# xmlyqing00/V-FloodNet

Hardware: AMD Instinct MI355X
Metric: segmented frames/sec at 480p (higher is better)
Workload: dtype f32

## Files before the change

### include/vfn_hip.h

```cpp
#ifndef VFN_HIP_H
#define VFN_HIP_H

#ifdef __cplusplus
extern "C" {
#endif

#define VFN_ABI_VERSION 18
enum { VFN_DESC_CONV = 0, VFN_DESC_STEM = 1, VFN_DESC_BANKSCAN = 2, VFN_DESC_MEMREAD = 3, VFN_DESC_BANK = 4, VFN_DESC_WGRAD = 5,
       VFN_DESC_REFRESH_FILTER = 6, VFN_DESC_REFRESH_EPILOGUE = 7, VFN_DESC_GATHER = 8, VFN_DESC_BANKMATCH = 9,
       VFN_DESC_TRAIN_AUG = 10 };
int vfn_abi_version(void);
int vfn_sizeof_desc(int which);

typedef struct vfn_conv_desc {
    const float* in;
    const float* w;
    const float* scale;
    const float* shift;
    const float* res;
    float* out;
    int N, H, W, Cin, in_ld;
    int Ho, Wo, Cout, cout_pad, out_ld, res_ld;
    int KH, KW, stride, pad;
    int relu_in, relu_out;
// ... 125 lines not shown
    const float* var;
    float* scale;
    float* shift;
    float eps;
    int C;
} vfn_refresh_epilogue;
int vfn_refresh_elems_per_block(void);
int vfn_refresh_filters_f32(const vfn_refresh_filter* table_dev, int n, int total_blocks, void* stream);
int vfn_refresh_epilogues_f32(const vfn_refresh_epilogue* table_dev, int n, void* stream);
typedef struct vfn_gather_entry {
    const float* src;
    long long dst_offset;
    long long stride[4];
    int shape[4];
    int block0;
    int reserved;
} vfn_gather_entry;
int vfn_gather_strided_f32(const vfn_gather_entry* table_dev, int n, int total_blocks, float* dst, void* stream);
int vfn_dilate2_f32(const float* g, float* out, int N, int Ho, int Wo, int H, int W, int C, void* stream);
int vfn_bn_param_grads_f32(const float* g, const float* y, const float* idn, const float* beta, const float* gamma, int M, int C,
                           float* partial, int nb, float* dgamma, float* dbeta, void* stream);
int vfn_bn_param_grads_acc_f32(const float* g, const float* y, const float* idn, const float* beta, const float* gamma, int M, int C,
                               float* partial, int nb, float* dgamma, float* dbeta, int accumulate, int* counter,
                               void* stream);
int vfn_maxpool3x3s2_backward_f32(const float* x, const float* g, float* gx, int N, int H, int W, int C, const float* add, int relu_mask,
                                  void* stream);
int vfn_softmax_cols_f32(const float* S, int B, int Q, int ld, float scale, float* P, void* stream);
int vfn_softmax_cols_backward_f32(const float* P, const float* dP, int B, int Q, int ld, float scale, float* dS, void* stream);
int vfn_adamw_f32(float* p, const float* g, float* m, float* v, long long n, double lr, double beta1, double beta2, double eps,
                  double weight_decay, int step, void* stream);
int vfn_colsum_f32(const float* x, int M, int C, int ld, float* partial, int nb, float* out, void* stream);
#define VFN_COLSUM_COUNTERS 64
int vfn_colsum_acc_f32(const float* x, int M, int C, int ld, float* partial, int nb, float* out, int accumulate, int* counter,
                       void* stream);
int vfn_upsample2x_add_backward_f32(const float* gm, float* gs, float* gpm, int N, int h, int w, int C, int s_bcast,
                                    void* stream);
int vfn_segment_loss_f32(const float* logit, const int* label, int bs, int obj_n, int n, float lu, float* partial, float* stats,
                         float* grad, void* stream);
int vfn_segment_uncertainty_backward_f32(const float* logit, int bs, int obj_n, int n, const float* g_unc_dev,
                                         const float* g_scores, float* partial, float* stats, float* grad, void* stream);
int vfn_tail_grad_o_f32(const float* G, const float* p_up, const float* unc, const float* conf, const float* q, float* g_o,
                        int obj_n, int h, int w, int pad_top, int pad_left, int H0, int W0, void* stream);
int vfn_tail_split_f32(const float* g_p2, const float* unc, const float* conf, const float* q, float* g_q, float* g_cf, float* g_u,
                       int obj_n, int npix, void* stream);
int vfn_local_stats_backward_f32(const float* g_lm, const float* lm, const float* g_cf, const float* g_u, const float* g_p2,
                                 const float* r1, const float* rough, const float* p_up, float* dA, float* dBv, int* amax,
                                 float* g_r1, float* g_pup, int obj_n, int h, int w, int C, void* stream);

typedef struct vfn_bankscan_desc {
    const float* q;
    const float* bank_k;
    const int* bank_len;
    const float* rowscale;
    float* part;
    long long stride_q, stride_k, stride_rs;
    float scale;
    int ldq, q_per_obj, HW, obj_n, nsplit, mode;
    int precision;
    int* work_counter;
    const void* bank_k_lp;
    float* scores;
    long long stride_scores;
} vfn_bankscan_desc;

typedef struct vfn_memread_desc {
    const float* q;
    const float* qv;
    const float* bank_k;
    const float* bank_v;
    const int* bank_len;
    const float* ml;
    float* o_part;
    int* cnt;
    float* info;
    float* out;
    long long stride_k, stride_v, stride_cnt, stride_info;
    float scale, thres;
    int ldq, ldqv, ld_out, HW, obj_n, nsplit;
    int precision;
    const void* bank_k_lp;
    const void* bank_v_lp;
    const float* scores;
    long long stride_scores;
} vfn_memread_desc;

int vfn_bank_scan(const vfn_bankscan_desc* d, void* stream);
int vfn_bank_scan_finish(const float* part, int nsplit, int HW, int obj_n, int mode, float* ml, int* idx,
                         float* corr, const float* colscale, void* stream);
int vfn_memread_apply(const vfn_memread_desc* d, void* stream);

typedef struct vfn_bankmatch_desc {
    const float* q;
    const float* bank_k;
    const void* bank_k_lp;
    const int* bank_len;
    const float* rowscale;
    const float* qnorm;
    const float* colscale;
    float* part_x3;
    float* part_f32;
    int* ulist;
    int* ucount;
    int* utotal;
    int* work_counter;
    int* match_idx;
    float* match_corr;
    long long stride_q, stride_k, stride_rs;
    int ldq, HW, obj_n;
    int nsplit;
    int nsplit_fb;
} vfn_bankmatch_desc;
int vfn_bank_match_certified(const vfn_bankmatch_desc* d, void* stream);
int vfn_memread_finish(const vfn_memread_desc* d, void* stream);

#define VFN_BANK_MAX_HW 32768
typedef struct vfn_bank_desc {
    float* bank_k;
    float* bank_v;
    float* info;
    float* scratch_k;
    float* scratch_v;
    float* scratch_info;
    const int* bank_len;
    int* bank_len_rw;
    const float* bank_knorm;
    const float* bank_vnorm;
    const int* match_idx;
    const float* match_corr;
    const float* new_k;
    const float* new_knorm;
    const float* new_vnorm;
    int* app_pos;
    int* keep_dst;
    int* plan;
    int* stats;
    long long stride_k, stride_v, stride_info, stride_n, stride_new;
    double class_budget;
    float thres_close, update_rate, new_hit_init;
    int frame_idx, ld_new, voff, HW, obj_n, cap;
    int rm_class;
    int rm_request;
} vfn_bank_desc;

int vfn_bank_refresh_lp(const vfn_bank_desc* d, void* bank_k_lp, void* bank_v_lp, int all_rows, void* stream);
int vfn_bank_refresh_lp_keys(const vfn_bank_desc* d, void* bank_k_lp, int all_rows, void* stream);

int vfn_row_norms(const float* x, long long stride_obj, int ld, int dim, const int* len_dev, int rows,
                  int obj_n, float* nrm, float* inv , long long stride_n, void* stream);
int vfn_bank_merge(const vfn_bank_desc* d, void* stream);
int vfn_bank_append(const vfn_bank_desc* d, void* stream);
int vfn_bank_remove(const vfn_bank_desc* d, void* stream);
int vfn_bank_refresh_norms(const vfn_bank_desc* d, float* bank_knorm, float* bank_kinv, float* bank_vnorm, void* stream);
int vfn_scatter_mean_f32(const float* src, long long src_s0, long long src_s1, const long long* index,
                         int S, float* out, long long out_s0, long long out_s1, int D, void* stream);
int vfn_scatter_mean_checked_f32(const float* src, long long src_s0, long long src_s1, const long long* index,
                                 long long index_s0, int S, float* out, long long out_s0, long long out_s1, int D,
                                 long long B, int* status, void* stream);

int vfn_resize_bicubic_f32(const float* in, float* out, int C, int Hi, int Wi, int Ho, int Wo, void* stream);
int vfn_resize_nearest_f32(const float* in, float* out, int C, int Hi, int Wi, int Ho, int Wo, void* stream);
int vfn_softmax_objects_f32(const float* score, float* prob, int obj_n, int n, void* stream);
int vfn_resize_argmax_u8(const float* prob, unsigned char* label, int obj_n, int Hi, int Wi, int Ho, int Wo,
                         void* stream);
int vfn_postprocess_pred_u8(const unsigned char* pred_host, int H, int W, unsigned char* out_host);
int vfn_postprocess_pred_device_u8(const unsigned char* pred, unsigned char* out, int* scratch, int H, int W,
                                   void* stream);
// ... 111 lines not shown
```

### v-floodnet_amd/csrc/memory_read.hip

```cpp
#include "common.h"
#include "../../include/vfn_hip.h"
#include <type_traits>
#include <cstdlib>

namespace {

constexpr int DK = 128, DV = 512;
constexpr int CH = 64;

__device__ __forceinline__ int swz(int row, int chunk) { return row * DK + ((chunk ^ (row & 15)) << 2); }

__device__ __forceinline__ int swz64(int row, int chunk) { return row * CH + ((chunk ^ (row & 15)) << 2); }

__device__ __forceinline__ void chunk_load_async(float* sK, const float* src, int valid, int wave, int lane) {
#pragma unroll
    for (int j = 0; j < 8; ++j) {
        const int r = (wave * 8 + j) * 2 + (lane >> 5);
        const int pc = lane & 31;
        const int rr = min(r, valid - 1);
        const float* g = src + (size_t)rr * DK + ((pc ^ (r & 15)) << 2);
        __builtin_amdgcn_global_load_lds(g, sK + (wave * 8 + j) * 2 * DK, 16, 0, 0);
    }
}

// ... 1331 lines not shown
    }

    PH_DECL;
    for (int c = c_lo; c < c_hi; ++c) {
        const int b0 = c * CH;
        const bool more = c + 1 < c_hi;

        f32x16 acc;
        score_tile(sK, sQ, wr, wq, li, lh, acc);
        PH_MARK(0);

        const int rloc = wr * 32 + 4 * lh;
        const int mycnt = softmax_hits(acc, p.scale, qm, qinv, p.thres, B - b0, rloc);
#pragma unroll
        for (int g = 0; g < 4; ++g) {
            const int brow = rloc + 8 * g;
            const f32x4 v = {acc[4 * g], acc[4 * g + 1], acc[4 * g + 2], acc[4 * g + 3]};
            *reinterpret_cast<f32x4*>(sP + swz64(qcol, brow >> 2)) = v;
        }
        if (p.cnt && lh == 0 && mycnt > 0) {
            const int row = b0 + wr * 32 + li;
            if (row < B) atomicAdd(p.cnt + (size_t)obj * p.stride_cnt + row, mycnt);
        }
        PH_MARK(1);
        __syncthreads();
        PH_MARK(2);
        if (more) chunk_load_async8(sK, K + (size_t)(b0 + CH) * DK, min(CH, B - b0 - CH), wave, lane);

        f32x2 vb[3][4];
        const __amdgpu_buffer_rsrc_t vrsrc = __builtin_amdgcn_make_buffer_rsrc(
            const_cast<float*>(V + (size_t)b0 * DV), 0, min(CH, B - b0) * DV * 4, 0x00020000);
        auto load_v = [&](int kk, int slot) {
#pragma unroll
            for (int t = 0; t < 4; ++t)
                vb[slot][t] = __builtin_bit_cast(f32x2, __builtin_amdgcn_raw_buffer_load_b64(vrsrc, vlane_off + (unsigned)((8 * kk + t) * DV * 4), 0, 0));
        };
        load_v(0, 0);
        load_v(1, 1);
        __builtin_amdgcn_sched_barrier(0);
#pragma unroll
        for (int kk = 0; kk < CH / 8; ++kk) {
            const int cur = kk % 3;
            if (kk + 2 < CH / 8) load_v(kk + 2, (kk + 2) % 3);
            __builtin_amdgcn_sched_barrier(0);
            const int lc = 2 * kk + lh;
            f32x4 a[4];
#pragma unroll
            for (int tq = 0; tq < 4; ++tq) a[tq] = *reinterpret_cast<const f32x4*>(sP + swz64(tq * 32 + li, lc));
#pragma unroll
            for (int t = 0; t < 4; ++t)
#pragma unroll
                for (int tq = 0; tq < 4; ++tq) {
                    o[tq][0] = __builtin_amdgcn_mfma_f32_32x32x2f32(a[tq][t], vb[cur][t][0], o[tq][0], 0, 0, 0);
                    o[tq][1] = __builtin_amdgcn_mfma_f32_32x32x2f32(a[tq][t], vb[cur][t][1], o[tq][1], 0, 0, 0);
                }
        }
        PH_MARK(3);
        __syncthreads();
        PH_MARK(4);
    }
#ifdef VFN_CENSUS
    if ((threadIdx.x & 63) == 0) {
        const int lin = (blockIdx.y * gridDim.x + blockIdx.x) * 8 + (threadIdx.x >> 6);
        if (lin < 2048) {
            for (int k = 0; k < 5; ++k) vfn_census_buf[lin * 8 + k] = ph_acc[k];
            vfn_census_buf[lin * 8 + 5] = c_hi - c_lo;
        }
    }
#endif

    float* dst = p.o_part + ((size_t)obj * p.nsplit + split) * p.HW * DV;
#pragma unroll
    for (int tq = 0; tq < 4; ++tq)
#pragma unroll
        for (int r = 0; r < 16; ++r) {
            const int q = q0 + tq * 32 + (r & 3) + 8 * (r >> 2) + 4 * lh;
            if (q < p.HW) {
                const f32x2 v = {o[tq][0][r], o[tq][1][r]};
                *reinterpret_cast<f32x2*>(dst + (size_t)q * DV + wave * 64 + li * 2) = v;
            }
        }
}

__global__ __launch_bounds__(512, 1)
void memread_apply_ss_kernel(const vfn_memread_desc p) {
    extern __shared__ __attribute__((aligned(16))) char smem[];
    float* sP = reinterpret_cast<float*>(smem);

    const int tid = threadIdx.x, lane = tid & 63, wave = tid >> 6;
    const int li = lane & 31, lh = lane >> 5;
    const int wr = wave >> 2, wq = wave & 3;
    int split, qt, obj, q0, B;
    apply_slice(p, split, qt, obj, q0, B);
    const int qtiles = (p.HW + QTW - 1) / QTW;
    const float* V = p.bank_v + (size_t)obj * p.stride_v;
    const float* S = p.scores + (size_t)obj * p.stride_scores;

    int c_lo, c_hi;
    chunk_range(B, p.nsplit, split, c_lo, c_hi);

    f32x16 o[4][2];
#pragma unroll
    for (int a = 0; a < 4; ++a)
#pragma unroll
        for (int b = 0; b < 2; ++b)
#pragma unroll
            for (int r = 0; r < 16; ++r) o[a][b][r] = 0.f;

    const unsigned vlane_off = (unsigned)((4 * lh) * DV + wave * 64 + li * 2) * 4u;
    const unsigned slane_off = (unsigned)(((wr * 4) * 2 + lh) * QTW + wq * 32 + li) * 16u;
    f32x4 sv[4];
    auto load_scores = [&](int c) {
        const char* tile = reinterpret_cast<const char*>(S + ((size_t)c * qtiles + qt) * (CH * QTW));
#pragma unroll
        for (int g = 0; g < 4; ++g) sv[g] = __builtin_nontemporal_load(reinterpret_cast<const f32x4*>(tile + slane_off + g * (2 * QTW * 16)));
    };
    const int qcol = wq * 32 + li;
    float qm, qinv;
    load_qstats(p, obj, q0, qcol, qm, qinv);
    const int rloc = wr * 32 + 4 * lh;
    auto softmax_to = [&](int c, float* sPb) {
        f32x16 acc;
#pragma unroll
        for (int r = 0; r < 16; ++r) acc[r] = sv[r >> 2][r & 3];
        const int b0 = c * CH;
        const int mycnt = softmax_hits(acc, p.scale, qm, qinv, p.thres, B - b0, rloc);
#pragma unroll
        for (int g = 0; g < 4; ++g) {
            const int brow = rloc + 8 * g;
            const f32x4 v = {acc[4 * g], acc[4 * g + 1], acc[4 * g + 2], acc[4 * g + 3]};
            *reinterpret_cast<f32x4*>(sPb + swz64(qcol, brow >> 2)) = v;
        }
        if (p.cnt && lh == 0 && mycnt > 0) {
            const int row = b0 + wr * 32 + li;
            if (row < B) atomicAdd(p.cnt + (size_t)obj * p.stride_cnt + row, mycnt);
        }
    };

    f32x2 vb[4][4];
    auto chunk_rsrc = [&](int c) {
        const int rows = c < c_hi ? min(CH, B - c * CH) : 0;
        return __builtin_amdgcn_make_buffer_rsrc(const_cast<float*>(V + (size_t)min(c, max(c_hi - 1, 0)) * CH * DV), 0, rows * DV * 4, 0x00020000);
    };
    auto load_v = [&](const __amdgpu_buffer_rsrc_t& rs, int kk, int slot) {
#pragma unroll
        for (int t = 0; t < 4; ++t)
            vb[slot][t] = __builtin_bit_cast(f32x2, __builtin_amdgcn_raw_buffer_load_b64(rs, vlane_off + (unsigned)((8 * kk + t) * DV * 4), 0, 0));
    };
    if (c_lo < c_hi) {
        const __amdgpu_buffer_rsrc_t rs0 = chunk_rsrc(c_lo);
        load_v(rs0, 0, 0);
        load_v(rs0, 1, 1);
        load_scores(c_lo);
        softmax_to(c_lo, sP);
        if (c_lo + 1 < c_hi) load_scores(c_lo + 1);
    }
    __syncthreads();

    for (int c = c_lo; c < c_hi; ++c) {
        const int b0 = c * CH;
        const int buf = (c - c_lo) & 1;
        const float* sPc = sP + buf * (QTW * CH);
        float* sPn = sP + (buf ^ 1) * (QTW * CH);
        const bool nxt = c + 1 < c_hi;

        const __amdgpu_buffer_rsrc_t vrsrc = chunk_rsrc(c), vrsrc_n = chunk_rsrc(c + 1);
        f32x4 a[2][4];
#pragma unroll
        for (int tq = 0; tq < 4; ++tq) a[0][tq] = *reinterpret_cast<const f32x4*>(sPc + swz64(tq * 32 + li, lh));
        __builtin_amdgcn_sched_barrier(0);
#pragma unroll
        for (int kk = 0; kk < CH / 8; ++kk) {
            const int cur = kk % 4;
            if (kk + 2 < CH / 8) load_v(vrsrc, kk + 2, (kk + 2) % 4);
            else load_v(vrsrc_n, kk + 2 - CH / 8, (kk + 2) % 4);
            if (kk + 1 < CH / 8) {
#pragma unroll
                for (int tq = 0; tq < 4; ++tq)
                    a[(kk + 1) & 1][tq] = *reinterpret_cast<const f32x4*>(sPc + swz64(tq * 32 + li, 2 * (kk + 1) + lh));
            }
            __builtin_amdgcn_sched_barrier(0);
#pragma unroll
            for (int t = 0; t < 4; ++t)
#pragma unroll
                for (int tq = 0; tq < 4; ++tq) {
                    o[tq][0] = __builtin_amdgcn_mfma_f32_32x32x2f32(a[kk & 1][tq][t], vb[cur][t][0], o[tq][0], 0, 0, 0);
                    o[tq][1] = __builtin_amdgcn_mfma_f32_32x32x2f32(a[kk & 1][tq][t], vb[cur][t][1], o[tq][1], 0, 0, 0);
                }
            if (kk == 2 && nxt) {
                softmax_to(c + 1, sPn);
                if (c + 2 < c_hi) load_scores(c + 2);
            }
        }
        __syncthreads();
    }

    float* dst = p.o_part + ((size_t)obj * p.nsplit + split) * p.HW * DV;
#pragma unroll
    for (int tq = 0; tq < 4; ++tq)
#pragma unroll
        for (int r = 0; r < 16; ++r) {
            const int q = q0 + tq * 32 + (r & 3) + 8 * (r >> 2) + 4 * lh;
            if (q < p.HW) {
                const f32x2 v = {o[tq][0][r], o[tq][1][r]};
                *reinterpret_cast<f32x2*>(dst + (size_t)q * DV + wave * 64 + li * 2) = v;
            }
        }
}

__global__ void memread_finish_kernel(const vfn_memread_desc p) {
    const int obj = blockIdx.y;
    const size_t total = (size_t)p.HW * (DV / 4);
    for (size_t i = blockIdx.x * (size_t)blockDim.x + threadIdx.x; i < total; i += (size_t)gridDim.x * blockDim.x) {
        const int c4 = i % (DV / 4);
        const int q = i / (DV / 4);
        f32x4 s = {0.f, 0.f, 0.f, 0.f};
        for (int sp = 0; sp < p.nsplit; ++sp)
            s += *reinterpret_cast<const f32x4*>(p.o_part + (((size_t)obj * p.nsplit + sp) * p.HW + q) * DV + c4 * 4);
        float* o = p.out + ((size_t)obj * p.HW + q) * p.ld_out;
        *reinterpret_cast<f32x4*>(o + c4 * 4) = s;
        if (p.qv) *reinterpret_cast<f32x4*>(o + DV + c4 * 4) = *reinterpret_cast<const f32x4*>(p.qv + (size_t)q * p.ldqv + c4 * 4);
    }
    if (p.cnt) {
        const int B = p.bank_len[obj];
        int* cnt = p.cnt + (size_t)obj * p.stride_cnt;
        float* info = p.info + (size_t)obj * p.stride_info;
        for (int b = blockIdx.x * blockDim.x + threadIdx.x; b < B; b += gridDim.x * blockDim.x) {
            info[(size_t)b * 2 + 1] += logf((float)cnt[b] + 1.f);
            cnt[b] = 0;
        }
    }
}

constexpr size_t SCAN_LDS = (size_t)(2 * CH * DK) * sizeof(float);

bool scores_fit(long long stride_scores, long long stride_k, int HW) {
    const long long cap = stride_k / DK;
    return stride_scores >= ((cap + CH - 1) / CH) * (long long)((HW + 127) / 128) * 8192;
}

template <typename K>
void allow_lds(K kern, size_t bytes) {
    hipFuncSetAttribute(reinterpret_cast<const void*>(kern), hipFuncAttributeMaxDynamicSharedMemorySize, (int)bytes);
}

int env_int(const char* name, int dflt) {
    const char* e = getenv(name);
    return e ? atoi(e) : dflt;
}

}

extern "C" int vfn_bank_scan(const vfn_bankscan_desc* d, void* stream) {
    if (!d || !d->q || !d->bank_k || !d->bank_len || !d->part) return VFN_ERR_ARG;
    if (d->nsplit < 1 || d->HW < 1 || d->obj_n < 1 || d->ldq % 4) return VFN_ERR_ARG;
    if (d->mode == 1 && (!d->rowscale || d->stride_rs % 4)) return VFN_ERR_ARG;
    if (d->precision < 0 || d->precision > 2) return VFN_ERR_ARG;
    if (d->scores && (d->mode != 0 || !scores_fit(d->stride_scores, d->stride_k, d->HW))) return VFN_ERR_ARG;
    static const int pipe_wgs = [] {
        allow_lds(bank_scan_kernel<0, 0>, SCAN_LDS); allow_lds(bank_scan_kernel<1, 0>, SCAN_LDS);
        allow_lds(bank_scan_kernel<0, 1>, SCAN_LDS); allow_lds(bank_scan_kernel<1, 1>, SCAN_LDS);
        allow_lds(bank_scan_kernel<0, 2>, SCAN_LDS); allow_lds(bank_scan_kernel<1, 2>, SCAN_LDS);
        const int wgs = env_int("VFN_SCAN_WGS", 768);
        return wgs < 1 ? 768 : wgs;
    }();
    if (!d->work_counter) return VFN_ERR_ARG;
    const int items = cdiv(d->HW, QTS) * d->nsplit * d->obj_n;
    hipStream_t s = (hipStream_t)stream;
    if (hipMemsetAsync(d->work_counter, 0, sizeof(int), s) != hipSuccess) return VFN_ERR_LAUNCH;
    const bool pipe = d->precision == 1 && d->bank_k_lp && env_int("VFN_SCAN_PIPE", 1) != 0;
    const int wgs = pipe ? pipe_wgs : 512;
    const dim3 grid(items < wgs ? items : wgs), block(256);
    auto scan = [&](auto kern) { hipLaunchKernelGGL(kern, grid, block, SCAN_LDS, s, *d, scan_gather{}); };
    if (pipe) {
        if (d->mode == 0) hipLaunchKernelGGL((bank_scan_pipe_kernel<0>), grid, block, SCAN_PIPE_LDS, s, *d);
        else hipLaunchKernelGGL((bank_scan_pipe_kernel<1>), grid, block, SCAN_PIPE_LDS, s, *d);
    } else if (d->mode == 0) {
        if (d->precision == 0) scan(bank_scan_kernel<0, 0>);
        else if (d->precision == 1) scan(bank_scan_kernel<0, 1>);
        else scan(bank_scan_kernel<0, 2>);
    } else if (d->mode == 1) {
        if (d->precision == 0) scan(bank_scan_kernel<1, 0>);
        else if (d->precision == 1) scan(bank_scan_kernel<1, 1>);
        else scan(bank_scan_kernel<1, 2>);
    } else {
        return VFN_ERR_ARG;
    }
    return vfn_check_launch();
}

extern "C" int vfn_bank_scan_finish(const float* part, int nsplit, int HW, int obj_n, int mode, float* ml, int* idx,
                                    float* corr, const float* colscale, void* stream) {
    if (!part) return VFN_ERR_ARG;
    const int total = obj_n * HW;
    if (mode == 0) {
        if (!ml) return VFN_ERR_ARG;
        hipLaunchKernelGGL(bank_scan_finish_kernel<0>, dim3(cdiv(total * 8, 256)), dim3(256), 0, (hipStream_t)stream,
                           part, nsplit, HW, obj_n, ml, idx, corr, colscale);
    } else {
        if (!idx || !corr || !colscale) return VFN_ERR_ARG;
        hipLaunchKernelGGL(bank_scan_finish_kernel<1>, dim3(cdiv(total * 8, 256)), dim3(256), 0, (hipStream_t)stream,
                           part, nsplit, HW, obj_n, ml, idx, corr, colscale);
    }
    return vfn_check_launch();
}

extern "C" int vfn_bank_match_certified(const vfn_bankmatch_desc* d, void* stream) {
    if (!d || !d->q || !d->bank_k || !d->bank_k_lp || !d->bank_len || !d->rowscale || !d->qnorm || !d->colscale) return VFN_ERR_ARG;
    if (!d->part_x3 || !d->part_f32 || !d->ulist || !d->ucount || !d->work_counter || !d->match_idx || !d->match_corr) return VFN_ERR_ARG;
    if (d->nsplit < 1 || d->nsplit_fb < 1 || d->HW < 1 || d->obj_n < 1 || d->ldq % 4 || d->stride_rs % 4) return VFN_ERR_ARG;
    static const bool ready = [] {
        allow_lds(bank_scan_kernel<2, 2>, SCAN_LDS); allow_lds(bank_scan_kernel<1, 0, true>, SCAN_LDS);
        return true;
    }();
    (void)ready;
    hipStream_t s = (hipStream_t)stream;
    vfn_bankscan_desc sd = {};
    sd.q = d->q; sd.bank_k = d->bank_k; sd.bank_len = d->bank_len; sd.rowscale = d->rowscale;
    sd.stride_q = d->stride_q; sd.stride_k = d->stride_k; sd.stride_rs = d->stride_rs;
    sd.scale = 1.f; sd.ldq = d->ldq; sd.q_per_obj = 1; sd.HW = d->HW; sd.obj_n = d->obj_n;
    sd.work_counter = d->work_counter; sd.bank_k_lp = d->bank_k_lp;
    sd.part = d->part_x3; sd.nsplit = d->nsplit; sd.mode = 2; sd.precision = 2;
    const int items = cdiv(d->HW, QTS) * d->nsplit * d->obj_n;
    if (hipMemsetAsync(d->work_counter, 0, sizeof(int), s) != hipSuccess) return VFN_ERR_LAUNCH;
    if (hipMemsetAsync(d->ucount, 0, sizeof(int) * d->obj_n, s) != hipSuccess) return VFN_ERR_LAUNCH;
    hipLaunchKernelGGL((bank_scan_kernel<2, 2>), dim3(items < 512 ? items : 512), dim3(256), SCAN_LDS, s, sd, scan_gather{});
    hipLaunchKernelGGL(bank_match_certify_kernel, dim3(cdiv(d->HW, 32), d->obj_n), dim3(64), 0, s, *d);
    sd.part = d->part_f32; sd.nsplit = d->nsplit_fb; sd.mode = 1; sd.precision = 0; sd.bank_k_lp = nullptr;
    if (hipMemsetAsync(d->work_counter, 0, sizeof(int), s) != hipSuccess) return VFN_ERR_LAUNCH;
    hipLaunchKernelGGL((bank_scan_kernel<1, 0, true>), dim3(512), dim3(256), SCAN_LDS, s, sd, scan_gather{d->ulist, d->ucount});
    hipLaunchKernelGGL(bank_match_finish_listed_kernel, dim3(cdiv(d->obj_n * d->HW * 8, 256)), dim3(256), 0, s,
                       (const float*)d->part_f32, d->nsplit_fb, d->HW, d->obj_n, (const int*)d->ulist, (const int*)d->ucount,
                       d->match_idx, d->match_corr, d->colscale);
    return vfn_check_launch();
}

extern "C" int vfn_memread_apply(const vfn_memread_desc* d, void* stream) {
    if (!d || !d->q || !d->bank_k || !d->bank_v || !d->bank_len || !d->ml || !d->o_part) return VFN_ERR_ARG;
    if (d->nsplit < 1 || d->ldq % 4) return VFN_ERR_ARG;
    if (d->precision < 0 || d->precision > 2) return VFN_ERR_ARG;
    if (d->scores && !scores_fit(d->stride_scores, d->stride_k, d->HW)) return VFN_ERR_ARG;
    constexpr size_t LDS_WF = (size_t)(QTW * DK + CH * DK + QTW * CH) * sizeof(float);
    constexpr size_t LDS_SS = (size_t)2 * QTW * CH * sizeof(float);
    constexpr size_t LDS_W1 = (size_t)QTW * DK * 2 + (size_t)CH * DK * 4 + 2 * (size_t)QTW * CH * 2;
    constexpr size_t LDS_W2 = LDS_W1 + (size_t)QTW * DK * 2;
    struct setup_t { int status; bool img_bf16; };
    static const setup_t setup = [] {
        allow_lds(memread_apply_wide_kernel, LDS_WF);
        allow_lds(memread_apply_lpw_kernel<false>, LDS_W1); allow_lds(memread_apply_lpw_kernel<true>, LDS_W2);
        allow_lds(memread_apply_shw_kernel<false>, LDS_W1); allow_lds(memread_apply_shw_kernel<true>, LDS_W2);
        allow_lds(memread_apply_pipe_kernel, APPLY_PIPE_LDS);
        const int lin = env_int("VFN_APPLY_XCD", 1) == 0 ? 1 : 0;
        const bool ok = !lin || hipMemcpyToSymbol(HIP_SYMBOL(vfn_apply_linear_order), &lin, sizeof(int)) == hipSuccess;
        return setup_t{ok ? VFN_OK : VFN_ERR_LAUNCH, env_int("VFN_APPLY_IMG_BF16", 1) != 0};
    }();
    if (setup.status != VFN_OK) return setup.status;

    const bool image = d->bank_k_lp && d->bank_v_lp && (d->precision == 2 || setup.img_bf16);
    void (*kern)(const vfn_memread_desc);
    size_t lds;
    if (d->precision == 0) {
        if (d->scores) { kern = memread_apply_ss_kernel; lds = LDS_SS; }
        else { kern = memread_apply_wide_kernel; lds = LDS_WF; }
    } else if (d->precision == 2) {
        kern = image ? memread_apply_shw_kernel<true> : memread_apply_lpw_kernel<true>; lds = LDS_W2;
    } else if (!image) {
        kern = memread_apply_lpw_kernel<false>; lds = LDS_W1;
    } else if (env_int("VFN_APPLY_PIPE", 1) != 0) {
        kern = memread_apply_pipe_kernel; lds = APPLY_PIPE_LDS;
    } else {
        kern = memread_apply_shw_kernel<false>; lds = LDS_W1;
    }
    const dim3 grid(cdiv(d->HW, QTW) * d->nsplit, d->obj_n);
    hipLaunchKernelGGL(kern, grid, dim3(512), lds, (hipStream_t)stream, *d);
    return vfn_check_launch();
}

extern "C" int vfn_memread_finish(const vfn_memread_desc* d, void* stream) {
    if (!d || !d->o_part || !d->out || !d->bank_len) return VFN_ERR_ARG;
    if (d->cnt && !d->info) return VFN_ERR_ARG;
    if (d->ld_out % 4 || d->ldqv % 4) return VFN_ERR_ARG;
    const dim3 grid(1024, d->obj_n);
    hipLaunchKernelGGL(memread_finish_kernel, grid, dim3(256), 0, (hipStream_t)stream, *d);
    return vfn_check_launch();
}

#ifdef VFN_CENSUS
extern "C" int vfn_debug_census(unsigned long long* host_out) {
    return hipMemcpyFromSymbol(host_out, HIP_SYMBOL(vfn_census_buf), sizeof(unsigned long long) * 4096 * 4) == hipSuccess ? 0 : 1;
}
#endif
```

### v-floodnet_amd/engine.py

```python
import math
import os

import torch

from . import _lib, ops, weights as W
from ._lib import ptr, stream, check, MemReadDesc, BankScanDesc
from .feature_bank import pick_nsplit, pick_scan_slices, MAX_SPLIT, MAX_SPLIT_SCAN, QT_SCAN, DK, DV

_CFG_EFF = {(128, 128): 1.00, (128, 64): 0.95, (64, 128): 0.95, (64, 64): 0.86, (32, 64): 0.74,
            (64, 32): 0.74, (128, 32): 0.80, (256, 128): 0.97}
_CFG_TILES = None
_TUNED = {}
_TUNED_PATH = __import__('os').path.join(__import__('os').path.dirname(__import__('os').path.abspath(__file__)),
                                         'tuned_gfx950.json')
_TUNED_BF16 = {}
_TUNED_BF16_PATH = _TUNED_PATH.replace('tuned_gfx950.json', 'tuned_gfx950_bf16.json')
_TUNED_BF16X3 = {}
_TUNED_BF16X3_PATH = _TUNED_PATH.replace('tuned_gfx950.json', 'tuned_gfx950_bf16x3.json')
_TABLES = (_TUNED, _TUNED_BF16, _TUNED_BF16X3)
_TABLE_PATHS = (_TUNED_PATH, _TUNED_BF16_PATH, _TUNED_BF16X3_PATH)
_TUNED_WINO6 = {}
_TUNED_WINO6_PATH = _TUNED_PATH.replace('tuned_gfx950.json', 'tuned_gfx950_wino6.json')
_TUNED_SHORTCUT = {}
_TUNED_SHORTCUT_PATH = _TUNED_PATH.replace('tuned_gfx950.json', 'tuned_gfx950_shortcut.json')
_TUNED_THIN = {}
_TUNED_THIN_PATH = _TUNED_PATH.replace('tuned_gfx950.json', 'tuned_gfx950_thin.json')


def is_wino6_desc(d):
    return d.w_batch_rows > 0 and d.M == 64 * d.w_batch_rows


def table_of(d, mode):
    return _TUNED_WINO6 if mode == 0 and is_wino6_desc(d) else _TABLES[mode]


def _load_tuned():
    import json
    import os
    if os.environ.get('VFN_IGNORE_TUNED') == '1':
        return
    for path, table in zip(_TABLE_PATHS + (_TUNED_WINO6_PATH,), _TABLES + (_TUNED_WINO6,)):
        alt = os.environ.get('VFN_TUNED_DIR')
        if alt and os.path.isfile(os.path.join(alt, os.path.basename(path))):
            path = os.path.join(alt, os.path.basename(path))
        if os.path.isfile(path):
            for k, v in json.load(open(path)).items():
                t = (int(v[0]), int(v[1]), int(v[2]) if len(v) > 2 else 0)
                table[tuple(int(x) for x in k.split(','))] = t + tuple(int(x) for x in v[3:6]) if len(v) >= 6 else t
    path = _TUNED_SHORTCUT_PATH
    alt = os.environ.get('VFN_TUNED_DIR')
    if alt and os.path.isfile(os.path.join(alt, os.path.basename(path))):
        path = os.path.join(alt, os.path.basename(path))
    if os.path.isfile(path):
        for k, v in json.load(open(path)).items():
            _TUNED_SHORTCUT[tuple(int(x) for x in k.split(','))] = (int(v[0]), int(v[1]))
    path = _TUNED_THIN_PATH
    if alt and os.path.isfile(os.path.join(alt, os.path.basename(path))):
        path = os.path.join(alt, os.path.basename(path))
    if os.path.isfile(path):
        for k, v in json.load(open(path)).items():
            _TUNED_THIN[tuple(int(x) for x in k.split(','))] = int(v)


def save_tuned(path=None, mode=0):
    import json
    if mode == 'thin':
        with open(path or _TUNED_THIN_PATH, 'w') as f:
            json.dump({','.join(str(x) for x in k): int(v) for k, v in sorted(_TUNED_THIN.items())}, f, indent=0)
        return
    table = _TUNED_WINO6 if mode == 'wino6' else _TUNED_SHORTCUT if mode == 'shortcut' else _TABLES[mode]
    with open(path or (_TUNED_WINO6_PATH if mode == 'wino6' else _TUNED_SHORTCUT_PATH if mode == 'shortcut' else _TABLE_PATHS[mode]), 'w') as f:
        json.dump({','.join(str(x) for x in k): list(v) for k, v in sorted(table.items())}, f, indent=0)


_load_tuned()


def pad_divide_by(h, w, d=16):
    new_h = h + d - h % d if h % d > 0 else h
    new_w = w + d - w % d if w % d > 0 else w
    lh = int((new_h - h) / 2)
    uh = int(new_h - h) - lh
    lw = int((new_w - w) / 2)
    uw = int(new_w - w) - lw
    return (lw, uw, lh, uh), new_h, new_w


WS_FLOATS = 16 * 1024 * 1024
_WINOGRAD_TRAIN = os.environ.get('VFN_WINOGRAD_TRAIN', '1') == '1'
# ... 1245 lines not shown
        assert n in (1, 2)
        p = self.plan(frames[0].shape[2], frames[0].shape[3], obj_n)
        if self.prefetch_pending(p):
            self.prefetch_finish(p)
        qs = self._idle_set(p)
        self.side_stream()
        ready = torch.cuda.Event()
        ready.record()
        with torch.cuda.stream(self._side):
            self._side.wait_event(ready)
            for i, fr in enumerate(frames):
                qs.frames[i].copy_(fr[0])
            lst = qs.pre[n]
            cut = len(lst) if full else qs.split[n]
            p.graphs.run(lst, 0, cut, eager=self.eager)
            qs.done = torch.cuda.Event()
            qs.done.record()
        self._side_busy = qs.done
        qs.keys = [self._key(fr) for fr in frames] + [None] * (2 - n)
        qs.held = list(frames) + [None] * (2 - n)
        qs.consumed = [False] * n + [True] * (2 - n)
        qs.n = n
        qs.stage = 2 if full else 1
        return True

    def prefetch_finish(self, p=None):
        plans = [p] if p is not None else list(self.plans.values())
        for pl in plans:
            for qs in pl.qsets:
                if qs.stage != 1:
                    continue
                ready = torch.cuda.Event()
                ready.record()
                with torch.cuda.stream(self._side):
                    self._side.wait_event(ready)
                    pl.graphs.run(qs.pre[qs.n], qs.split[qs.n], None, eager=self.eager)
                    qs.done = torch.cuda.Event()
                    qs.done.record()
                self._side_busy = qs.done
                qs.stage = 2

    def side_stream(self):
        if self._side is None:
            self._side = _lib.independent_stream(self.device)
        return self._side

    def prefetch_query(self, frame, obj_n):
        return self.prefetch_begin([frame], obj_n, full=True)

    def _memory_read(self, p, fb, update_bank, kv_q=None, out=None):
        L = _lib.lib()
        s = stream()
        kv_q = p.kv_q if kv_q is None else kv_q
        out = p.dec_in if out is None else out
        K, HW, cap = fb.obj_n, p.HW, fb._cap
        nsplit_scan = pick_scan_slices(HW, K, fb.len_upper())
        scale = 1.0 / math.sqrt(DK)
        d = BankScanDesc()
        d.q, d.bank_k, d.bank_len, d.rowscale, d.part = ptr(kv_q), ptr(fb._kbuf), ptr(fb._len_dev), None, ptr(p.ml_part)
        d.stride_q, d.stride_k, d.stride_rs = 0, cap * DK, 0
        d.scale = scale
        d.ldq, d.q_per_obj, d.HW, d.obj_n, d.nsplit, d.mode = DK + DV, 0, HW, K, nsplit_scan, 0
        mr_mode = self.layer_mode('memread') if hasattr(self, 'layer_mode') else self.mode
        d.precision = mr_mode
        d.work_counter = ptr(p.work)
        klp, vlp = fb.lp_image() if mr_mode else (None, None)
        d.bank_k_lp = ptr(klp) if klp is not None else None
        scores = _scores_buffer(p, fb) if mr_mode == 0 else None
        if scores is not None:
            d.scores, d.stride_scores = ptr(scores), scores.shape[1]
        check(L.vfn_bank_scan(_lib.C.byref(d), s), 'vfn_bank_scan')
        check(L.vfn_bank_scan_finish(ptr(p.ml_part), nsplit_scan, HW, K, 0, ptr(p.ml), None, None, None, s),
              'vfn_bank_scan_finish')
        m = MemReadDesc()
        m.q = ptr(kv_q)
        m.qv = None
        m.bank_k, m.bank_v, m.bank_len, m.ml, m.o_part = ptr(fb._kbuf), ptr(fb._vbuf), ptr(fb._len_dev), ptr(p.ml), ptr(p.o_part)
        m.cnt = ptr(fb._cnt) if update_bank else None
        m.info, m.out = ptr(fb._ibuf), ptr(out)
        m.stride_k, m.stride_v, m.stride_cnt, m.stride_info = cap * DK, cap * DV, cap, cap * 2
        m.scale, m.thres = scale, 1e-3
        m.ldq, m.ldqv, m.ld_out, m.HW, m.obj_n = DK + DV, DK + DV, out.shape[-1], HW, K
        m.precision = mr_mode
        m.nsplit = pick_nsplit(HW, K, fb.len_upper(), QT_SCAN, MAX_SPLIT)
        if klp is not None:
            m.bank_k_lp, m.bank_v_lp = ptr(klp), ptr(vlp)
        if scores is not None:
            m.scores, m.stride_scores = ptr(scores), scores.shape[1]
        check(L.vfn_memread_apply(_lib.C.byref(m), s), 'vfn_memread_apply')
        check(L.vfn_memread_finish(_lib.C.byref(m), s), 'vfn_memread_finish')

    def capture(self, H0, W0, obj_n, group=0):
        p = self.plan(H0, W0, obj_n)
        if not _GRAPHS or self.eager or p.keep_acts:
            return 0
        before = p.graphs.captures
        torch.cuda.current_stream().synchronize()
        p.graphs.warm(p.mem)
        for qs in p.qsets:
            for n in qs.sizes:
                lst = qs.pre[n]
                p.graphs.warm(lst)
                if 0 < qs.split[n] < len(lst):
                    p.graphs.warm(lst, 0, qs.split[n])
                    p.graphs.warm(lst, qs.split[n], None)
            for L in qs.post:
                p.graphs.warm(L)
        for G in ([group] if group and group > 1 else []):
            qs = p.batch_set(G)
            b = qs.dec_batch()
            if self.refresher._tables is None:
                self._settle()
            p.graphs.warm(qs.pre[G])
            p.graphs.warm(b.post)
        torch.cuda.current_stream().synchronize()
        return p.graphs.captures - before

    def autotune(self, H0, W0, obj_n, iters=3, only_missing=False, shape_filter=None, cfg_filter=None):
        p = self.plan(H0, W0, obj_n)
        seen = {}
        side_sets = list(p.qsets) + ([] if p.keep_acts else list(p._qbatch.values()))
        side_lists = [id(qs.pre[n]) for qs in side_sets for n in qs.sizes]
        for lst in p.all_lists():
            for l in lst:
                l_side = id(lst) in side_lists
                if l.fn is ops.conv2d_launch:
                    d = l.args[0]
                    if ops.is_thin3x3_cfg(l.args[1]):
                        continue
                    key = (d.M, d.Cout, d.KH * d.KW * d.Cin, int(l.args[2]), is_wino6_desc(d))
                    if only_missing and key[:3] in table_of(d, key[3]):
                        continue
                    if shape_filter is not None and not shape_filter(key[:3]):
                        continue
                    seen.setdefault(key, []).append((l, l_side))
        for key, launches in seen.items():
            d = launches[0][0].args[0]
            bf = key[3]
            if key[4]:
                best = tune_desc(d, bf, p.ws, p.cnt, iters=iters, cfg_filter=lambda k_, c_: c_ >= ops.WINO_GEMM_CFG0 and (cfg_filter is None or cfg_filter(k_, c_)))
            else:
                best = tune_desc(d, bf, p.ws, p.cnt, iters=iters, cfg_filter=cfg_filter)
            table_of(d, bf)[key[:3]] = best
            for l, in_q in launches:
                l.args = (l.args[0], apply_choice(l.args[0], best, p.ws_q if in_q else p.ws, p.cnt_q if in_q else p.cnt), bf)
        if seen:
            p.graphs.invalidate()
        return dict(_TABLES[self.mode])
```

### v-floodnet_amd/feature_bank.py

```python
import numpy as np
import torch

from . import _lib, ops
from ._lib import ptr, stream, check, BankDesc, BankScanDesc, BankMatchDesc

DK, DV = 128, 512
MAX_SPLIT = 20
MAX_SPLIT_SCAN = 256
QT, QT_SCAN, CH = 64, 128, 64
MAX_HW = _lib.DEFINES['VFN_BANK_MAX_HW']


def pick_scan_slices(hw, obj_n, b_upper, target_items=1536, min_chunks=8):
    nchunks = max(1, (b_upper + CH - 1) // CH)
    qtiles = (hw + QT_SCAN - 1) // QT_SCAN
    import os
    if os.environ.get('VFN_NSPLIT_SCAN'):
        return max(1, min(int(os.environ['VFN_NSPLIT_SCAN']), nchunks, MAX_SPLIT_SCAN))
    want = max(1, target_items // (qtiles * obj_n))
    return max(1, min(want, nchunks // min_chunks if nchunks >= min_chunks else 1, MAX_SPLIT_SCAN))


def pick_fallback_slices(obj_n, b_upper, target_items=512, min_chunks=4):
    nchunks = max(1, (b_upper + CH - 1) // CH)
    return max(1, min(target_items // obj_n, nchunks // min_chunks, MAX_SPLIT_SCAN))


def pick_nsplit(hw, obj_n, b_upper, qt=QT, max_split=MAX_SPLIT):
    nchunks = max(1, (b_upper + CH - 1) // CH)
    qtiles = (hw + qt - 1) // qt
    import os
    env = 'VFN_NSPLIT' if qt == QT else 'VFN_NSPLIT_SCAN'
    if os.environ.get(env):
        return min(int(os.environ[env]), nchunks, max_split)
    best, best_eff = 1, -1.0
    for s in range(1, max(1, min(nchunks // 3, max_split)) + 1):
        blocks = qtiles * obj_n * s
        eff = blocks / (((blocks + 255) // 256) * 256)
        if eff >= best_eff:
            best, best_eff = s, eff
    return best


class FeatureBank:
    def __init__(self, obj_n, memory_budget, device, update_rate=0.1, thres_close=0.95, precision=None):
        self.obj_n = obj_n
        self.update_rate = update_rate
        self.thres_close = thres_close
        self.device = torch.device(device)
        import os
        self.precision = precision or os.environ.get('VFN_PRECISION', 'fp32')
        if self.precision not in ops.MODES:
            raise ValueError(f'precision must be one of {sorted(ops.MODES)}, got {self.precision!r}')

        self._graph_kv = None
        self.peak_n = np.zeros(obj_n)
        self.replace_n = np.zeros(obj_n)

        self.class_budget = memory_budget // obj_n
        if obj_n == 2:
            self.class_budget = 0.8 * self.class_budget

        self._cap = 0
        self._hw = 0
        self._len_host = None
        self._len_upper = None
        self._n_updates = 0
        self._hist = {}
        self._dirty = False
        self._kbuf = self._vbuf = self._ibuf = None
        self._scratch = None
        self._norms_valid = self._lp_valid = False
        self._klp = self._vlp = None
        self._kimg_valid = False
        self._mbuf = None
        self._match_updates = 0

    def _require_gpu(self):
        if self.device.type != 'cuda':
            raise RuntimeError('FeatureBank lives in GPU memory (HIP kernels only, no CPU fallback); '
                               f'got device {self.device}')
        _lib.lib()

    def _alloc(self, hw, n_init):
        self._require_gpu()
        dev = self.device
        o = self.obj_n
        cap = (int(max(self.class_budget, n_init)) + 2 * hw + 2 * CH + 63) // 64 * 64
        self._cap, self._hw = cap, hw
        self._kbuf = torch.empty(o, cap, DK, device=dev)
        self._vbuf = torch.empty(o, cap, DV, device=dev)
        self._ibuf = torch.zeros(o, cap, 2, device=dev)
        self._len_dev = torch.zeros(o, dtype=torch.int32, device=dev)
        self._stats = torch.zeros(o, 4, dtype=torch.int32, device=dev)
        self._knorm = torch.empty(o, cap, device=dev)
        self._vnorm = torch.empty(o, cap, device=dev)
        self._kinv = torch.empty(o, cap, device=dev)
        self._cnt = torch.zeros(o, cap, dtype=torch.int32, device=dev)
        self._keep_dst = torch.empty(o, cap, dtype=torch.int32, device=dev)
        self._plan = torch.zeros(o, 4, dtype=torch.int32, device=dev)
        self._new = torch.empty(o, hw, DK + DV, device=dev)
        self._nknorm = torch.empty(o, hw, device=dev)
        self._nvnorm = torch.empty(o, hw, device=dev)
        self._nkinv = torch.empty(o, hw, device=dev)
        self._midx = torch.empty(o, hw, dtype=torch.int32, device=dev)
        self._mcorr = torch.empty(o, hw, device=dev)
        self._app_pos = torch.empty(o, hw, dtype=torch.int32, device=dev)
        self._part = torch.empty(o, MAX_SPLIT_SCAN, hw, 2, device=dev)
        self._work = torch.zeros(4, dtype=torch.int32, device=dev)
        self._stats_pinned = torch.zeros(o, 4, dtype=torch.int32).pin_memory()
        self._scratch = None
        self._klp = self._vlp = None
        self._mbuf = None
        self._match_updates = 0
        self._norms_valid = self._lp_valid = self._kimg_valid = False

    def _ensure_scratch(self):
        if self._scratch is None:
            self._scratch = (torch.empty_like(self._kbuf), torch.empty_like(self._vbuf), torch.empty_like(self._ibuf))
        return self._scratch

    def _bank_desc(self):
        o, cap = self.obj_n, self._cap
        bd = BankDesc()
# ... 366 lines not shown
```

Measured before the change: 172.3.

## Give partial last query tile its own split count and trim dead MFMA work

The memory-read apply kernel now lets the last, partially filled query tile use a separate split count (nsplit_tail). It is templated on the number of live 32-row query sub-tiles, so the tail skips MFMAs and softmax for empty rows. A host-side cost model picks the main and tail split counts to balance work across CUs, and the finish kernel sums only the splits that the tail actually wrote. This adds template instantiations and a more complex grid mapping. The payoff depends on HW at 480p leaving a partial tile.

```diff
diff --git a/include/vfn_hip.h b/include/vfn_hip.h
--- a/include/vfn_hip.h
+++ b/include/vfn_hip.h
@@ -231,6 +231,7 @@
     const void* bank_v_lp;
     const float* scores;
     long long stride_scores;
+    int nsplit_tail;
 } vfn_memread_desc;
 
 int vfn_bank_scan(const vfn_bankscan_desc* d, void* stream);
diff --git a/v-floodnet_amd/csrc/memory_read.hip b/v-floodnet_amd/csrc/memory_read.hip
--- a/v-floodnet_amd/csrc/memory_read.hip
+++ b/v-floodnet_amd/csrc/memory_read.hip
@@ -1437,26 +1437,22 @@
         }
 }
 
-__global__ __launch_bounds__(512, 1)
-void memread_apply_ss_kernel(const vfn_memread_desc p) {
-    extern __shared__ __attribute__((aligned(16))) char smem[];
-    float* sP = reinterpret_cast<float*>(smem);
-
+template <int LIVE>
+__device__ __forceinline__ void apply_ss_item(const vfn_memread_desc& p, float* sP, int split, int nslices, int qt, int obj, int q0, int B) {
     const int tid = threadIdx.x, lane = tid & 63, wave = tid >> 6;
     const int li = lane & 31, lh = lane >> 5;
     const int wr = wave >> 2, wq = wave & 3;
-    int split, qt, obj, q0, B;
-    apply_slice(p, split, qt, obj, q0, B);
+    const bool smx = LIVE == 4 || wq < LIVE;
     const int qtiles = (p.HW + QTW - 1) / QTW;
     const float* V = p.bank_v + (size_t)obj * p.stride_v;
     const float* S = p.scores + (size_t)obj * p.stride_scores;
 
     int c_lo, c_hi;
-    chunk_range(B, p.nsplit, split, c_lo, c_hi);
-
-    f32x16 o[4][2];
-#pragma unroll
-    for (int a = 0; a < 4; ++a)
+    chunk_range(B, nslices, split, c_lo, c_hi);
+
+    f32x16 o[LIVE][2];
+#pragma unroll
+    for (int a = 0; a < LIVE; ++a)
 #pragma unroll
         for (int b = 0; b < 2; ++b)
 #pragma unroll
@@ -1506,9 +1502,11 @@
         const __amdgpu_buffer_rsrc_t rs0 = chunk_rsrc(c_lo);
         load_v(rs0, 0, 0);
         load_v(rs0, 1, 1);
-        load_scores(c_lo);
-        softmax_to(c_lo, sP);
-        if (c_lo + 1 < c_hi) load_scores(c_lo + 1);
+        if (smx) {
+            load_scores(c_lo);
+            softmax_to(c_lo, sP);
+            if (c_lo + 1 < c_hi) load_scores(c_lo + 1);
+        }
     }
     __syncthreads();
 
@@ -1520,9 +1518,9 @@
         const bool nxt = c + 1 < c_hi;
 
         const __amdgpu_buffer_rsrc_t vrsrc = chunk_rsrc(c), vrsrc_n = chunk_rsrc(c + 1);
-        f32x4 a[2][4];
-#pragma unroll
-        for (int tq = 0; tq < 4; ++tq) a[0][tq] = *reinterpret_cast<const f32x4*>(sPc + swz64(tq * 32 + li, lh));
+        f32x4 a[2][LIVE];
+#pragma unroll
+        for (int tq = 0; tq < LIVE; ++tq) a[0][tq] = *reinterpret_cast<const f32x4*>(sPc + swz64(tq * 32 + li, lh));
         __builtin_amdgcn_sched_barrier(0);
 #pragma unroll
         for (int kk = 0; kk < CH / 8; ++kk) {
@@ -1531,18 +1529,18 @@
             else load_v(vrsrc_n, kk + 2 - CH / 8, (kk + 2) % 4);
             if (kk + 1 < CH / 8) {
 #pragma unroll
-                for (int tq = 0; tq < 4; ++tq)
+                for (int tq = 0; tq < LIVE; ++tq)
                     a[(kk + 1) & 1][tq] = *reinterpret_cast<const f32x4*>(sPc + swz64(tq * 32 + li, 2 * (kk + 1) + lh));
             }
             __builtin_amdgcn_sched_barrier(0);
 #pragma unroll
             for (int t = 0; t < 4; ++t)
 #pragma unroll
-                for (int tq = 0; tq < 4; ++tq) {
+                for (int tq = 0; tq < LIVE; ++tq) {
                     o[tq][0] = __builtin_amdgcn_mfma_f32_32x32x2f32(a[kk & 1][tq][t], vb[cur][t][0], o[tq][0], 0, 0, 0);
                     o[tq][1] = __builtin_amdgcn_mfma_f32_32x32x2f32(a[kk & 1][tq][t], vb[cur][t][1], o[tq][1], 0, 0, 0);
                 }
-            if (kk == 2 && nxt) {
+            if (kk == 2 && nxt && smx) {
                 softmax_to(c + 1, sPn);
                 if (c + 2 < c_hi) load_scores(c + 2);
             }
@@ -1552,7 +1550,7 @@
 
     float* dst = p.o_part + ((size_t)obj * p.nsplit + split) * p.HW * DV;
 #pragma unroll
-    for (int tq = 0; tq < 4; ++tq)
+    for (int tq = 0; tq < LIVE; ++tq)
 #pragma unroll
         for (int r = 0; r < 16; ++r) {
             const int q = q0 + tq * 32 + (r & 3) + 8 * (r >> 2) + 4 * lh;
@@ -1563,14 +1561,55 @@
         }
 }
 
+__device__ __forceinline__ void apply_tail_item(const vfn_memread_desc& p, int qtiles, int& split, int& qt, int& obj) {
+    const int per_obj = (int)gridDim.x;
+    int L = (int)blockIdx.x;
+    obj = (int)blockIdx.y;
+    if (!vfn_apply_linear_order) {
+        const int total = (int)(gridDim.x * gridDim.y);
+        const int id = (int)(blockIdx.y * gridDim.x + blockIdx.x);
+        const int q = total >> 3, r = total & 7;
+        const int xcd = id & 7, slot = id >> 3;
+        L = (xcd < r ? xcd * (q + 1) : r * (q + 1) + (xcd - r) * q) + slot;
+        obj = L / per_obj;
+        L -= obj * per_obj;
+    }
+    const int full = (qtiles - 1) * p.nsplit;
+    if (L < full) { split = L / (qtiles - 1); qt = L - split * (qtiles - 1); }
+    else { split = L - full; qt = qtiles - 1; }
+}
+
+__global__ __launch_bounds__(512, 1)
+void memread_apply_ss_kernel(const vfn_memread_desc p) {
+    extern __shared__ __attribute__((aligned(16))) char smem[];
+    float* sP = reinterpret_cast<float*>(smem);
+    int split, qt, obj, q0, B;
+    if (p.nsplit_tail <= 0) {
+        apply_slice(p, split, qt, obj, q0, B);
+        apply_ss_item<4>(p, sP, split, p.nsplit, qt, obj, q0, B);
+        return;
+    }
+    const int qtiles = (p.HW + QTW - 1) / QTW;
+    apply_tail_item(p, qtiles, split, qt, obj);
+    q0 = qt * QTW;
+    B = p.bank_len[obj];
+    const int live = qt == qtiles - 1 ? (p.HW - q0 + 31) >> 5 : 4;
+    if (live == 4) apply_ss_item<4>(p, sP, split, qt == qtiles - 1 ? p.nsplit_tail : p.nsplit, qt, obj, q0, B);
+    else if (live == 3) apply_ss_item<3>(p, sP, split, p.nsplit_tail, qt, obj, q0, B);
+    else if (live == 2) apply_ss_item<2>(p, sP, split, p.nsplit_tail, qt, obj, q0, B);
+    else apply_ss_item<1>(p, sP, split, p.nsplit_tail, qt, obj, q0, B);
+}
+
 __global__ void memread_finish_kernel(const vfn_memread_desc p) {
     const int obj = blockIdx.y;
     const size_t total = (size_t)p.HW * (DV / 4);
+    const int last_q0 = (p.HW - 1) / QTW * QTW;
     for (size_t i = blockIdx.x * (size_t)blockDim.x + threadIdx.x; i < total; i += (size_t)gridDim.x * blockDim.x) {
         const int c4 = i % (DV / 4);
         const int q = i / (DV / 4);
         f32x4 s = {0.f, 0.f, 0.f, 0.f};
-        for (int sp = 0; sp < p.nsplit; ++sp)
+        const int ns = p.nsplit_tail > 0 && q >= last_q0 ? p.nsplit_tail : p.nsplit;
+        for (int sp = 0; sp < ns; ++sp)
             s += *reinterpret_cast<const f32x4*>(p.o_part + (((size_t)obj * p.nsplit + sp) * p.HW + q) * DV + c4 * 4);
         float* o = p.out + ((size_t)obj * p.HW + q) * p.ld_out;
         *reinterpret_cast<f32x4*>(o + c4 * 4) = s;
@@ -1695,6 +1734,8 @@
     if (d->nsplit < 1 || d->ldq % 4) return VFN_ERR_ARG;
     if (d->precision < 0 || d->precision > 2) return VFN_ERR_ARG;
     if (d->scores && !scores_fit(d->stride_scores, d->stride_k, d->HW)) return VFN_ERR_ARG;
+    if (d->nsplit_tail < 0 || d->nsplit_tail > d->nsplit) return VFN_ERR_ARG;
+    if (d->nsplit_tail && !(d->precision == 0 && d->scores)) return VFN_ERR_ARG;
     constexpr size_t LDS_WF = (size_t)(QTW * DK + CH * DK + QTW * CH) * sizeof(float);
     constexpr size_t LDS_SS = (size_t)2 * QTW * CH * sizeof(float);
     constexpr size_t LDS_W1 = (size_t)QTW * DK * 2 + (size_t)CH * DK * 4 + 2 * (size_t)QTW * CH * 2;
@@ -1726,7 +1767,8 @@
     } else {
         kern = memread_apply_shw_kernel<false>; lds = LDS_W1;
     }
-    const dim3 grid(cdiv(d->HW, QTW) * d->nsplit, d->obj_n);
+    const int qtiles = cdiv(d->HW, QTW);
+    const dim3 grid(d->nsplit_tail > 0 ? (qtiles - 1) * d->nsplit + d->nsplit_tail : qtiles * d->nsplit, d->obj_n);
     hipLaunchKernelGGL(kern, grid, dim3(512), lds, (hipStream_t)stream, *d);
     return vfn_check_launch();
 }
@@ -1735,6 +1777,7 @@
     if (!d || !d->o_part || !d->out || !d->bank_len) return VFN_ERR_ARG;
     if (d->cnt && !d->info) return VFN_ERR_ARG;
     if (d->ld_out % 4 || d->ldqv % 4) return VFN_ERR_ARG;
+    if (d->nsplit_tail < 0 || d->nsplit_tail > d->nsplit) return VFN_ERR_ARG;
     const dim3 grid(1024, d->obj_n);
     hipLaunchKernelGGL(memread_finish_kernel, grid, dim3(256), 0, (hipStream_t)stream, *d);
     return vfn_check_launch();
diff --git a/v-floodnet_amd/engine.py b/v-floodnet_amd/engine.py
--- a/v-floodnet_amd/engine.py
+++ b/v-floodnet_amd/engine.py
@@ -5,7 +5,7 @@
 
 from . import _lib, ops, weights as W
 from ._lib import ptr, stream, check, MemReadDesc, BankScanDesc
-from .feature_bank import pick_nsplit, pick_scan_slices, MAX_SPLIT, MAX_SPLIT_SCAN, QT_SCAN, DK, DV
+from .feature_bank import pick_nsplit, pick_apply_split, pick_scan_slices, MAX_SPLIT, MAX_SPLIT_SCAN, QT_SCAN, DK, DV
 
 _CFG_EFF = {(128, 128): 1.00, (128, 64): 0.95, (64, 128): 0.95, (64, 64): 0.86, (32, 64): 0.74,
             (64, 32): 0.74, (128, 32): 0.80, (256, 128): 0.97}
@@ -1417,7 +1417,10 @@
         m.scale, m.thres = scale, 1e-3
         m.ldq, m.ldqv, m.ld_out, m.HW, m.obj_n = DK + DV, DK + DV, out.shape[-1], HW, K
         m.precision = mr_mode
-        m.nsplit = pick_nsplit(HW, K, fb.len_upper(), QT_SCAN, MAX_SPLIT)
+        if mr_mode == 0 and scores is not None:
+            m.nsplit, m.nsplit_tail = pick_apply_split(HW, K, fb.len_upper())
+        else:
+            m.nsplit = pick_nsplit(HW, K, fb.len_upper(), QT_SCAN, MAX_SPLIT)
         if klp is not None:
             m.bank_k_lp, m.bank_v_lp = ptr(klp), ptr(vlp)
         if scores is not None:
diff --git a/v-floodnet_amd/feature_bank.py b/v-floodnet_amd/feature_bank.py
--- a/v-floodnet_amd/feature_bank.py
+++ b/v-floodnet_amd/feature_bank.py
@@ -40,6 +40,43 @@
         if eff >= best_eff:
             best, best_eff = s, eff
     return best
+
+
+APPLY_TAIL_WEIGHT = {3: 1.01, 2: 1.05, 1: 1.23}
+CUS = 256
+
+
+def apply_split_cost(hw, obj_n, nchunks, nsplit, nsplit_tail):
+    qtiles = (hw + QT_SCAN - 1) // QT_SCAN
+    full = -(-nchunks // nsplit) * 4.0
+    if nsplit_tail == 0:
+        return -(-qtiles * obj_n * nsplit // CUS) * full
+    live = -(-(hw - (qtiles - 1) * QT_SCAN) // 32)
+    tail = -(-nchunks // nsplit_tail) * live * APPLY_TAIL_WEIGHT.get(live, 4.0 / live)
+    wgs = obj_n * ((qtiles - 1) * nsplit + nsplit_tail)
+    return -(-wgs // CUS) * (max(full, tail) if qtiles > 1 else tail)
+
+
+def pick_apply_split(hw, obj_n, b_upper):
+    import os
+    nchunks = max(1, (b_upper + CH - 1) // CH)
+    qtiles = (hw + QT_SCAN - 1) // QT_SCAN
+    live = -(-(hw - (qtiles - 1) * QT_SCAN) // 32)
+    uniform = pick_nsplit(hw, obj_n, b_upper, QT_SCAN, MAX_SPLIT)
+    if os.environ.get('VFN_APPLY_TAIL', '1') == '0':
+        return uniform, 0
+    if os.environ.get('VFN_APPLY_SPLIT'):
+        s, t = (int(x) for x in os.environ['VFN_APPLY_SPLIT'].split(','))
+        s = max(1, min(s, MAX_SPLIT))
+        return s, max(0, min(t, s))
+    if live not in APPLY_TAIL_WEIGHT:
+        return uniform, 0
+    smax = max(1, min(nchunks // 3, MAX_SPLIT))
+    cands = [(apply_split_cost(hw, obj_n, nchunks, s, t), s, t) for s in range(1, smax + 1) for t in range(1, s + 1)]
+    least = min(c for c, _, _ in cands)
+    bar = min(1.01 * least, max(least, apply_split_cost(hw, obj_n, nchunks, uniform, 0)))
+    _, s, t = min((c for c in cands if c[0] <= bar), key=lambda c: (c[1], c[0], c[2]))
+    return s, t
 
 
 class FeatureBank:
```

Result: faster. 174.8, median of 6 (+1.5%).
